# openclimatefix/predict_pv_yield

Measured on AMD Instinct MI355X. Metric: PV-site samples/sec (train step), conv3d 12->6 frames, higher is better.
Workload: dtype bf16; 1 GPU; conv3d train step (fwd + NMAE + bwd + Adam): sat [B,11,18,64,64] N(0,1), 4x Conv3d(3x3x3, 32ch) + fc 128/128/64, 128.6 M params; per_gpu_batch=32, global_batch=32, t_frames=18, parallelism=single

## Files before the change

### predict_pv_yield_amd/csrc/conv3d_wgrad_bf16_v2.hip

```cpp
#include "pv_common.h"

namespace pv {

constexpr int W2TR = 8, W2TRI = 10, W2TW = 32, W2XW = 34;
constexpr int W2_SLAB_ELEMS = 28 * 32 * 32;
constexpr uint32_t W2_INVALID = 0x40000000u;

typedef __attribute__((address_space(3))) s16x4 w2_lds_s16x4;
typedef __attribute__((address_space(3))) unsigned char* w2_lds_ptr;
typedef int w2_i32x4 __attribute__((ext_vector_type(4)));

__device__ __forceinline__ void w2_lds_dma16(uint32_t lds_addr, uint32_t voff, w2_i32x4 rsrc, uint32_t soff) {
  asm volatile("s_mov_b32 m0, %0\n\ts_nop 0\n\tbuffer_load_dwordx4 %1, %2, %3 offen lds" ::"s"(lds_addr), "v"(voff), "s"(rsrc),
               "s"(soff)
               : "memory");
}
__device__ __forceinline__ w2_i32x4 w2_rsrc(const void* base, int bytes) {
  const uintptr_t a = (uintptr_t)base;
  return (w2_i32x4){(int)(uint32_t)a, (int)((a >> 32) & 0xffffu), bytes, 0x00020000};
}

#ifdef PV_DIAG_STAMPS
__device__ unsigned long long wgrad2_diag[PV_DIAG_WAVES * PV_DIAG_SLOTS];
#endif

template <int NACC, int Q>
__device__ __forceinline__ void w2_interleave() {
  if constexpr (Q < NACC) {
    constexpr int R = 2 + 2 * NACC;
    __builtin_amdgcn_sched_group_barrier(0x008, 1, 0);
    __builtin_amdgcn_sched_group_barrier(0x100, R / NACC + (Q < R % NACC ? 1 : 0), 0);
    w2_interleave<NACC, Q + 1>();
  }
}

template <int CPAD, bool F16 = false, bool PACK12 = false>
__global__ __launch_bounds__(512, 2) void conv3d_wgrad_bf16_v2_kernel(
    const uint16_t* __restrict__ x, const uint16_t* __restrict__ dy, float* __restrict__ slabs, int t_in, int h_in, int w_in,
    int t_out, int h_out, int w_out, int pad_t, int pad_h, int pad_w, int n_colblk, int t_chunk, int rpb) {
  constexpr int NCH = CPAD / 8;
  constexpr int VPR = 16 / NCH;
  constexpr int VOXB = CPAD * 2;
  constexpr int ROWB = W2XW * VOXB;
  constexpr int SLOTB = W2TRI * ROWB;
  constexpr int XVPP = 1024 / VOXB;
  constexpr int XPIECES = (W2XW + XVPP - 1) / XVPP;
  constexpr int XTAIL_LANES = (W2XW - (XPIECES - 1) * XVPP) * NCH;
  constexpr int DROWB = W2TW * 64;
  constexpr int DSLOTB = W2TR * DROWB;
  constexpr int NXS = 5;
  __shared__ __attribute__((aligned(1024))) unsigned char lds[NXS * SLOTB + 256 + 2 * DSLOTB];
  unsigned char* lds_const = lds + NXS * SLOTB;
  unsigned char* lds_dy = lds_const + 256;

  const int tid = threadIdx.x;
  const int lane = tid & 63;
  const int wave8 = __builtin_amdgcn_readfirstlane(tid >> 6);
  const bool loader = wave8 >= 4;
  const int wave = wave8 & 3;
  const int grp = lane >> 4;
  const int qi = (lane & 15) >> 2;
  const int pi = lane & 3;
  const int hh = grp >> 1;
  const int cb = 16 * (grp & 1);

  const int h0 = blockIdx.x * rpb;
  const int b = blockIdx.z;
  const int tc0 = blockIdx.y * t_chunk;
  const int tc1 = min(tc0 + t_chunk, t_out);
  const int wg_id = (blockIdx.z * gridDim.y + blockIdx.y) * gridDim.x + blockIdx.x;
  float* slab = slabs + (size_t)wg_id * W2_SLAB_ELEMS;

  static_assert(!PACK12 || CPAD == 16, "PACK12 packs the 16-channel image");
  constexpr bool PAIRED = CPAD == 16;
  constexpr int NACC = PACK12 ? 3 : (PAIRED ? 4 : 7);
  f32x16 acc[NACC];
#pragma unroll
  for (int i = 0; i < NACC; ++i)
#pragma unroll
    for (int j = 0; j < 16; ++j) acc[i][j] = 0.f;

  const int nt = tc1 - tc0, tn = nt + 2;
  const int n_items = nt > 0 ? nt * n_colblk : 0;
  const int u_end = tn * n_colblk;
  const uint32_t lds_base = __builtin_amdgcn_readfirstlane((uint32_t)(uintptr_t)(w2_lds_ptr)lds);

  if (n_items > 0 && loader) {
    const uint32_t x_plane_b = (uint32_t)h_in * w_in * CPAD * 2u, x_row_b = (uint32_t)w_in * CPAD * 2u;
    const uint32_t d_plane_b = (uint32_t)h_out * w_out * 64u, d_row_b = (uint32_t)w_out * 64u;
    const size_t x_sample = (size_t)t_in * h_in * w_in * CPAD, d_sample = (size_t)t_out * h_out * w_out * 32;
    const void* const x_base = x + (size_t)b * x_sample;
    const void* const d_base = dy + (size_t)b * d_sample;
    const int x_bytes = (int)(x_sample * 2), d_bytes = (int)(d_sample * 2);
    uint32_t xrow_src[3];
    bool xrow_in[3];
#pragma unroll
    for (int i = 0; i < 3; ++i) {
      const int hi = h0 - pad_h + wave + 4 * i;
      xrow_in[i] = (unsigned)hi < (unsigned)h_in && wave + 4 * i < rpb + 2;
      xrow_src[i] = xrow_in[i] ? (uint32_t)hi * x_row_b : 0u;
    }
    uint32_t drow_src[2];
    bool drow_in[2];
#pragma unroll
    for (int i = 0; i < 2; ++i) {
      const int ho = h0 + wave + 4 * i;
      drow_in[i] = ho < h_out && wave + 4 * i < rpb;
      drow_src[i] = drow_in[i] ? (uint32_t)ho * d_row_b : 0u;
    }
    const bool has_third_row = wave + 8 < W2TRI;
    auto x_slice = [&](int u) {
      const int cb = u / tn, s = tc0 + (u - cb * tn), w0 = cb * W2TW;
      const int ti = s - pad_t;
      const bool t_ok = (unsigned)ti < (unsigned)t_in;
      const uint32_t slot = lds_base + (uint32_t)((u % NXS) * SLOTB);
#pragma unroll
      for (int pc = 0; pc < XPIECES; ++pc) {
        const int v = pc * XVPP + lane / NCH;
        const int src = (lane % NCH) ^ ((v / VPR) % NCH);
        const int wi = w0 - pad_w + v;
        const uint32_t lane_off = ((unsigned)wi < (unsigned)w_in && v < W2XW) ? (uint32_t)(wi * CPAD + src * 8) * 2u : W2_INVALID;
#pragma unroll
        for (int i = 0; i < 3; ++i) {
          if (i == 2 && !has_third_row) continue;
          const bool ok = t_ok && xrow_in[i];
          if (pc + 1 < XPIECES || lane < XTAIL_LANES)
            w2_lds_dma16(slot + (uint32_t)((wave + 4 * i) * ROWB + pc * 1024), lane_off, w2_rsrc(x_base, ok ? x_bytes : 0),
                         ok ? (uint32_t)ti * x_plane_b + xrow_src[i] : 0u);
        }
      }
    };
    auto d_slice = [&](int v_seq) {
      const int cb = v_seq / nt, t = tc0 + (v_seq - cb * nt), w0 = cb * W2TW;
      const uint32_t slot = lds_base + (uint32_t)(NXS * SLOTB + 256 + (v_seq & 1) * DSLOTB);
#pragma unroll
      for (int pc = 0; pc < 2; ++pc) {
        const int v = pc * 16 + (lane >> 2);
        const int src = (lane & 3) ^ ((v >> 2) & 3);
        const uint32_t lane_off = (w0 + v) < w_out ? (uint32_t)((w0 + v) * 32 + src * 8) * 2u : W2_INVALID;
#pragma unroll
        for (int i = 0; i < 2; ++i) {
          const bool ok = drow_in[i];
          w2_lds_dma16(slot + (uint32_t)((wave + 4 * i) * DROWB + pc * 1024), lane_off, w2_rsrc(d_base, ok ? d_bytes : 0),
                       ok ? (uint32_t)t * d_plane_b + drow_src[i] : 0u);
        }
      }
    };

    int next_u = 0;
    for (; next_u < 4 && next_u < u_end; ++next_u) x_slice(next_u);
    d_slice(0);
    for (int j = 0; j < n_items; ++j) {
      const int cb = j / nt, u0 = cb * tn + (j - cb * nt);
      __builtin_amdgcn_s_waitcnt(0x0f70);
      __syncthreads();
      if (next_u < u0 + 3) {
        for (; next_u < u0 + 3; ++next_u) x_slice(next_u);
        __builtin_amdgcn_s_waitcnt(0x0f70);
        __syncthreads();
      }
      for (; next_u <= u0 + 4 && next_u < u_end; ++next_u) x_slice(next_u);
      if (j + 1 < n_items) d_slice(j + 1);
    }
  } else if (n_items > 0) {
    if (tid < 64) reinterpret_cast<uint32_t*>(lds_const)[tid] = tid < 32 ? (F16 ? 0x3c003c00u : 0x3f803f80u) : 0u;

    int aoff[2];
#pragma unroll
    for (int s = 0; s < 2; ++s) {
      const int v = 8 * hh + 4 * s + qi;
      const int chunk = (cb + 4 * pi) >> 3;
      aoff[s] = v * 64 + ((chunk ^ ((v >> 2) & 3)) << 4) + (pi & 1) * 8;
    }
    int boff[NACC][2];
    int bkt[NACC];
    int my_tap[NACC];
#pragma unroll
    for (int i = 0; i < NACC; ++i) {
      int tap, c4 = 0;
      if constexpr (PACK12) {
        const int piece = 8 * (wave + 4 * i) + 4 * (grp & 1) + pi;
        tap = piece / 3;
        c4 = piece - 3 * tap;
        if (piece > 81) tap = 28;
      } else {
        tap = PAIRED ? 2 * (wave + 4 * i) + (grp & 1) : wave + 4 * i;
      }
      my_tap[i] = tap;
      if (tap > 26) tap = 26;
      const int kt = tap / 9, kh = (tap / 3) % 3, kw = tap % 3;
      bkt[i] = kt;
      const int cbx = PAIRED ? 0 : cb;
#pragma unroll
      for (int s = 0; s < 2; ++s) {
        const int v = kw + 8 * hh + 4 * s + qi;
        const int chunk = PACK12 ? (c4 >> 1) : ((cbx + 4 * pi) >> 3);
        const int sub = PACK12 ? (c4 & 1) : (pi & 1);
        boff[i][s] = kh * ROWB + v * VOXB + ((chunk ^ ((v / VPR) % NCH)) << 4) + sub * 8;
      }
    }
    typedef __attribute__((ext_vector_type(8))) short s16x8;
    const int last_tap = (PAIRED || PACK12) ? my_tap[NACC - 1] : (wave == 3 ? 27 : 0);
    const unsigned char* const_frag = last_tap < 27 ? nullptr : lds_const + (last_tap == 27 ? 0 : 128) + (lane & 15) * 8;

#ifdef PV_DIAG_STAMPS
    unsigned long long dg[PV_DIAG_SLOTS] = {0, 0, 0, 0, 0, 0, 0, 0}, s0, s1, s2;
#endif
    for (int j = 0; j < n_items; ++j) {
      const int cbj = j / nt, u0 = cbj * tn + (j - cbj * nt);
      PV_STAMP(s0);
      __syncthreads();
      if (cbj > 0 && j == cbj * nt) __syncthreads();
      PV_STAMP(s1);
      int slot_of_kt[3];
#pragma unroll
      for (int kt = 0; kt < 3; ++kt) slot_of_kt[kt] = ((u0 + kt) % NXS) * SLOTB;
      const unsigned char* dy_slot = lds_dy + (j & 1) * DSLOTB;
      int bslot[NACC];
#pragma unroll
      for (int i = 0; i < NACC; ++i) bslot[i] = bkt[i] == 0 ? slot_of_kt[0] : (bkt[i] == 1 ? slot_of_kt[1] : slot_of_kt[2]);
      auto read_step = [&](int st, s16x4 (&ra)[2], s16x4 (&rb)[NACC][2]) {
        const int rho = st >> 1, cg = st & 1;
        const unsigned char* ap = dy_slot + rho * DROWB + cg * 16 * 64;
        ra[0] = __builtin_amdgcn_ds_read_tr16_b64_v4i16((w2_lds_s16x4*)(ap + aoff[0]));
        ra[1] = __builtin_amdgcn_ds_read_tr16_b64_v4i16((w2_lds_s16x4*)(ap + aoff[1]));
        const int xo = rho * ROWB + cg * 16 * VOXB;
#pragma unroll
        for (int i = 0; i < NACC; ++i) {
          const unsigned char* bp = lds + bslot[i] + xo;
          const unsigned char* p0 = bp + boff[i][0];
          const unsigned char* p1 = bp + boff[i][1];
          if (i == NACC - 1) {
            p0 = const_frag ? const_frag : p0;
            p1 = const_frag ? const_frag : p1;
          }
          rb[i][0] = __builtin_amdgcn_ds_read_tr16_b64_v4i16((w2_lds_s16x4*)p0);
          rb[i][1] = __builtin_amdgcn_ds_read_tr16_b64_v4i16((w2_lds_s16x4*)p1);
        }
      };
      auto mfma_step = [&](const s16x4 (&ra)[2], const s16x4 (&rb)[NACC][2]) {
        const s16x8 a8 = {ra[0][0], ra[0][1], ra[0][2], ra[0][3], ra[1][0], ra[1][1], ra[1][2], ra[1][3]};
        typedef _Float16 w2_f16x8 __attribute__((ext_vector_type(8)));
#pragma unroll
        for (int i = 0; i < NACC; ++i) {
          s16x8 t8 = {rb[i][0][0], rb[i][0][1], rb[i][0][2], rb[i][0][3], rb[i][1][0], rb[i][1][1], rb[i][1][2], rb[i][1][3]};
          if constexpr (F16)
            acc[i] = __builtin_amdgcn_mfma_f32_32x32x16_f16(__builtin_bit_cast(w2_f16x8, a8), __builtin_bit_cast(w2_f16x8, t8), acc[i], 0, 0, 0);
          else
            acc[i] = __builtin_amdgcn_mfma_f32_32x32x16_bf16(__builtin_bit_cast(bf16x8, a8), __builtin_bit_cast(bf16x8, t8), acc[i], 0, 0, 0);
        }
      };
      s16x4 ra0[2], ra1[2], rb0[NACC][2], rb1[NACC][2];
      const bool skip_last_row = rpb < W2TR;
      read_step(0, ra0, rb0);
#pragma unroll
      for (int st = 0; st < W2TR * 2; st += 2) {
        if (st == W2TR * 2 - 2 && skip_last_row) break;
        __builtin_amdgcn_sched_barrier(0);
        read_step(st + 1, ra1, rb1);
        mfma_step(ra0, rb0);
        w2_interleave<NACC, 0>();
        __builtin_amdgcn_sched_barrier(0);
        if (st + 2 < W2TR * 2) {
          read_step(st + 2, ra0, rb0);
          mfma_step(ra1, rb1);
          w2_interleave<NACC, 0>();
        } else {
          mfma_step(ra1, rb1);
        }
        __builtin_amdgcn_sched_barrier(0);
      }
#ifdef PV_DIAG_STAMPS
      PV_STAMP(s2);
      dg[0] += s1 - s0;
      dg[1] += s2 - s1;
      dg[2] += 1;
#endif
    }
#ifdef PV_DIAG_STAMPS
    if (lane == 0 && wg_id * 4 + wave < PV_DIAG_WAVES)
      for (int i = 0; i < PV_DIAG_SLOTS; ++i) wgrad2_diag[(size_t)(wg_id * 4 + wave) * PV_DIAG_SLOTS + i] = dg[i];
#endif
  }
  if (loader) return;

  const int half = lane >> 5;
#pragma unroll
  for (int i = 0; i < NACC; ++i) {
    int tapslot = PAIRED ? 2 * (wave + 4 * i) + ((lane & 31) >> 4) : wave + 4 * i;
    int ci = PAIRED ? (lane & 15) : (lane & 31);
    if constexpr (PACK12) {
      const int piece = 8 * (wave + 4 * i) + ((lane & 31) >> 2);
      tapslot = piece / 3;
      ci = 4 * (piece - 3 * tapslot) + (lane & 3);
      if (piece > 81) tapslot = 28;
    }
    if (tapslot <= 27) {
      float* dst = slab + (size_t)tapslot * 1024 + ci;
#pragma unroll
      for (int j = 0; j < 16; ++j) {
        const int co = (j & 3) + 8 * (j >> 2) + 4 * half;
        dst[co * 32] = acc[i][j];
      }
    }
  }
}

void wgrad_v2_grid(const pv_conv3d_dims* d, int* n_rowblk, int* n_colblk, int* n_tchunk, int* t_chunk, int* rows_per_blk) {
  const int to = d->t_in + 2 * d->pad_t - 2, ho = d->h_in + 2 * d->pad_h - 2, wo = d->w_in + 2 * d->pad_w - 2;
  *n_rowblk = (ho + W2TR - 1) / W2TR;
  if ((long long)d->batch * *n_rowblk < 256 && (long long)d->batch * (*n_rowblk + 1) <= 256 &&
      (ho + *n_rowblk) / (*n_rowblk + 1) < (ho + *n_rowblk - 1) / *n_rowblk)
    *n_rowblk += 1;
  *rows_per_blk = (ho + *n_rowblk - 1) / *n_rowblk;
  *n_colblk = (wo + W2TW - 1) / W2TW;
  const long long tiles = (long long)d->batch * *n_rowblk;
  int max_chunks = (to + 1) / 2;
  if (max_chunks < 1) max_chunks = 1;
  int ntc = 1;
  long long best = -1;
  for (int c = 1; c <= max_chunks && tiles * c <= 16 * 256; ++c) {
    const int tch = (to + c - 1) / c, nch = (to + tch - 1) / tch;
    const long long rounds = (tiles * nch + 255) / 256;
    const long long cost = rounds * (tch + 2);
    if (best < 0 || cost < best) best = cost, ntc = nch;
  }
  *t_chunk = (to + ntc - 1) / ntc;
  *n_tchunk = (to + *t_chunk - 1) / *t_chunk;
}

size_t wgrad_v2_workspace_bytes(const pv_conv3d_dims* d) {
  int nrb, ncb, ntc, tch, rpb;
  wgrad_v2_grid(d, &nrb, &ncb, &ntc, &tch, &rpb);
  return (size_t)d->batch * nrb * ntc * W2_SLAB_ELEMS * sizeof(float);
}

int launch_conv3d_wgrad_bf16_v2(const uint16_t* x, const uint16_t* dy, float* slabs, const pv_conv3d_dims* d, int to, int ho,
                                int wo, hipStream_t st, int* n_slabs, bool f16) {
  if (((uintptr_t)x % 16) != 0 || ((uintptr_t)dy % 16) != 0) return 1;
  int nrb, ncb, ntc, tch, rpb;
  wgrad_v2_grid(d, &nrb, &ncb, &ntc, &tch, &rpb);
  *n_slabs = d->batch * nrb * ntc;
  dim3 grid((unsigned)nrb, (unsigned)ntc, (unsigned)d->batch);
#define PV_W2(CP, HALF)                                                                                                       \
  hipLaunchKernelGGL((conv3d_wgrad_bf16_v2_kernel<CP, HALF>), grid, dim3(512), 0, st, x, dy, slabs, d->t_in, d->h_in, d->w_in, to, \
                     ho, wo, d->pad_t, d->pad_h, d->pad_w, ncb, tch, rpb)
#define PV_W2P(HALF)                                                                                                        \
  hipLaunchKernelGGL((conv3d_wgrad_bf16_v2_kernel<16, HALF, true>), grid, dim3(512), 0, st, x, dy, slabs, d->t_in, d->h_in, d->w_in, \
                     to, ho, wo, d->pad_t, d->pad_h, d->pad_w, ncb, tch, rpb)
  if (pv_bf16_cpad(d->c_in) == 16) {
    const bool pack12 = d->c_in <= 12 && !getenv("PV_WGRAD_NO_PACK12");
    if (pack12) { if (f16) PV_W2P(true); else PV_W2P(false); }
    else { if (f16) PV_W2(16, true); else PV_W2(16, false); }
  } else { if (f16) PV_W2(32, true); else PV_W2(32, false); }
#undef PV_W2P
#undef PV_W2
  return 0;
}


constexpr int WR_GROUPS = 16;
__global__ __launch_bounds__(64 * WR_GROUPS) void conv3d_wgrad_reduce_kernel(const float* __restrict__ slabs, int n_slabs,
                                                                              float* __restrict__ dw, float* __restrict__ dbias,
                                                                              int c_out, int c_in) {
  __shared__ float part[WR_GROUPS][64];
  const int lane = threadIdx.x & 63, grp = threadIdx.x >> 6;
  const int i = blockIdx.x * 64 + lane;
  float s0 = 0.f, s1 = 0.f, s2 = 0.f, s3 = 0.f;
  for (int k = grp; k < n_slabs; k += 16 * WR_GROUPS) {
    float v[16];
#pragma unroll
    for (int j = 0; j < 16; ++j) v[j] = (k + WR_GROUPS * j < n_slabs) ? slabs[(size_t)(k + WR_GROUPS * j) * W2_SLAB_ELEMS + i] : 0.f;
#pragma unroll
    for (int j = 0; j < 16; j += 4) s0 += v[j], s1 += v[j + 1], s2 += v[j + 2], s3 += v[j + 3];
  }
  part[grp][lane] = (s0 + s1) + (s2 + s3);
  __syncthreads();
  if (grp == 0) {
    float t[WR_GROUPS];
#pragma unroll
    for (int q = 0; q < WR_GROUPS; ++q) t[q] = part[q][lane];
#pragma unroll
    for (int w = WR_GROUPS / 2; w >= 1; w >>= 1)
#pragma unroll
      for (int q = 0; q < w; ++q) t[q] = t[2 * q] + t[2 * q + 1];
    const float s = t[0];
    const int tap = i >> 10, co = (i >> 5) & 31, ci = i & 31;
    if (tap < 27) {
      if (dw && co < c_out && ci < c_in) dw[((size_t)co * c_in + ci) * 27 + tap] = s;
    } else if (dbias && ci == 0 && co < c_out) {
      dbias[co] = s;
    }
  }
}

__global__ __launch_bounds__(256) void wgrad_gate_copy_kernel(const u32x4* __restrict__ dy, const u32x4* __restrict__ y,
                                                              u32x4* __restrict__ dst, size_t n8) {
  const size_t stride = (size_t)gridDim.x * blockDim.x;
  for (size_t i = (size_t)blockIdx.x * blockDim.x + threadIdx.x; i < n8; i += stride) {
    const u32x4 g = dy[i], a = y[i];
    u32x4 o;
#pragma unroll
    for (int j = 0; j < 4; ++j) o[j] = g[j] & (relu_pair01(a[j]) * 0xffffu);
    dst[i] = o;
  }
}

}

using namespace pv;

extern "C" {

int pv_conv3d_bwd_weight_bf16_workspace_bytes(const pv_conv3d_dims* d, size_t* bytes) {
  PV_REQUIRE(d && bytes, PV_EINVAL, "pv_conv3d_bwd_weight_bf16_workspace_bytes: null pointer");
  PV_REQUIRE(d->batch > 0 && d->t_in > 0 && d->h_in > 0 && d->w_in > 0, PV_EINVAL,
             "pv_conv3d_bwd_weight_bf16_workspace_bytes: bad dims");
  const long long to = d->t_in + 2 * d->pad_t - 2, ho = d->h_in + 2 * d->pad_h - 2, wo = d->w_in + 2 * d->pad_w - 2;
  const size_t dy_bytes = (to > 0 && ho > 0 && wo > 0) ? (size_t)d->batch * to * ho * wo * pv_bf16_cpad(d->c_out) * 2 : 0;
  *bytes = ((wgrad_v2_workspace_bytes(d) + 255) & ~(size_t)255) + dy_bytes;
  return PV_OK;
}

int pv_conv3d_bwd_weight_bf16(const uint16_t* x, const uint16_t* dy, const uint16_t* y_relu_mask, float* dw,
                              float* dbias, const pv_conv3d_dims* d, void* workspace, size_t workspace_bytes,
                              void* stream) {
  PV_REQUIRE(d && x && dy && workspace, PV_EINVAL, "pv_conv3d_bwd_weight_bf16: null pointer");
  PV_REQUIRE(d->batch > 0 && d->c_in > 0 && d->c_in <= 32 && d->c_out > 0 && d->c_out <= 32, PV_ESIZE,
             "pv_conv3d_bwd_weight_bf16: channels (%d -> %d) must be in 1..32", d->c_in, d->c_out);
  PV_REQUIRE(d->pad_t >= 0 && d->pad_t <= 2 && d->pad_h >= 0 && d->pad_h <= 2 && d->pad_w >= 0 && d->pad_w <= 2,
             PV_EINVAL, "pv_conv3d_bwd_weight_bf16: padding must be 0..2");
  const int to = d->t_in + 2 * d->pad_t - 2, ho = d->h_in + 2 * d->pad_h - 2, wo = d->w_in + 2 * d->pad_w - 2;
  PV_REQUIRE(to > 0 && ho > 0 && wo > 0, PV_ESIZE, "pv_conv3d_bwd_weight_bf16: input smaller than the kernel");
  PV_REQUIRE(d->batch <= 65535, PV_ESIZE, "pv_conv3d_bwd_weight_bf16: batch too large for grid.z");
  PV_REQUIRE((size_t)d->t_in * d->h_in * d->w_in * 64 <= 0x40000000ull, PV_ESIZE,
             "pv_conv3d_bwd_weight_bf16: one sample exceeds 1 GiB (buffer-addressing limit of this kernel)");
  const size_t slab_bytes = (wgrad_v2_workspace_bytes(d) + 255) & ~(size_t)255;
  PV_REQUIRE(workspace_bytes >= wgrad_v2_workspace_bytes(d), PV_ESIZE, "pv_conv3d_bwd_weight_bf16: workspace too small");
  PV_REQUIRE(((uintptr_t)x % 16) == 0 && ((uintptr_t)dy % 16) == 0 && ((uintptr_t)workspace % 16) == 0, PV_EINVAL,
             "pv_conv3d_bwd_weight_bf16: x, dy and the workspace must be 16-byte aligned");
  hipStream_t st = as_stream(stream);
  if (y_relu_mask) {
    const size_t n = (size_t)d->batch * to * ho * wo * pv_bf16_cpad(d->c_out);
    PV_REQUIRE(workspace_bytes >= slab_bytes + n * 2, PV_ESIZE,
               "pv_conv3d_bwd_weight_bf16: a gate needs room for the gated copy of dY behind the slabs (workspace_bytes query)");
    PV_REQUIRE(((uintptr_t)y_relu_mask % 16) == 0, PV_EINVAL, "pv_conv3d_bwd_weight_bf16: the gate must be 16-byte aligned");
    uint16_t* gated = reinterpret_cast<uint16_t*>(static_cast<char*>(workspace) + slab_bytes);
    hipLaunchKernelGGL(wgrad_gate_copy_kernel, dim3(stream_grid(n / 8, 256)), dim3(256), 0, st,
                       reinterpret_cast<const u32x4*>(dy), reinterpret_cast<const u32x4*>(y_relu_mask),
                       reinterpret_cast<u32x4*>(gated), n / 8);
    dy = gated;
  }
  int n2 = 0;
  PV_REQUIRE(launch_conv3d_wgrad_bf16_v2(x, dy, (float*)workspace, d, to, ho, wo, st, &n2, false) == 0, PV_EINVAL,
             "pv_conv3d_bwd_weight_bf16: x and dy must be 16-byte aligned");
  hipLaunchKernelGGL(conv3d_wgrad_reduce_kernel, dim3(W2_SLAB_ELEMS / 64), dim3(64 * WR_GROUPS), 0, st, (const float*)workspace, n2,
                     dw, dbias, d->c_out, d->c_in);
  return check_launch("pv_conv3d_bwd_weight_bf16");
}

int pv_conv3d_bwd_weight_f16(const uint16_t* x, const uint16_t* dy, float* dw, float* dbias, const pv_conv3d_dims* d,
                             void* workspace, size_t workspace_bytes, void* stream) {
  PV_REQUIRE(d && x && dy && workspace, PV_EINVAL, "pv_conv3d_bwd_weight_f16: null pointer");
  PV_REQUIRE(d->batch > 0 && d->c_in > 0 && d->c_in <= 32 && d->c_out > 0 && d->c_out <= 32, PV_ESIZE,
             "pv_conv3d_bwd_weight_f16: channels (%d -> %d) must be in 1..32", d->c_in, d->c_out);
  PV_REQUIRE(d->pad_t >= 0 && d->pad_t <= 2 && d->pad_h >= 0 && d->pad_h <= 2 && d->pad_w >= 0 && d->pad_w <= 2,
             PV_EINVAL, "pv_conv3d_bwd_weight_f16: padding must be 0..2");
  const int to = d->t_in + 2 * d->pad_t - 2, ho = d->h_in + 2 * d->pad_h - 2, wo = d->w_in + 2 * d->pad_w - 2;
  PV_REQUIRE(to > 0 && ho > 0 && wo > 0, PV_ESIZE, "pv_conv3d_bwd_weight_f16: input smaller than the kernel");
  PV_REQUIRE(d->batch <= 65535, PV_ESIZE, "pv_conv3d_bwd_weight_f16: batch too large for grid.z");
  PV_REQUIRE((size_t)d->t_in * d->h_in * d->w_in * 64 <= 0x40000000ull, PV_ESIZE,
             "pv_conv3d_bwd_weight_f16: one sample exceeds 1 GiB (buffer-addressing limit of this kernel)");
  PV_REQUIRE(workspace_bytes >= wgrad_v2_workspace_bytes(d), PV_ESIZE, "pv_conv3d_bwd_weight_f16: workspace too small");
  hipStream_t st = as_stream(stream);
  int n2 = 0;
  PV_REQUIRE(launch_conv3d_wgrad_bf16_v2(x, dy, (float*)workspace, d, to, ho, wo, st, &n2, true) == 0, PV_EINVAL,
             "pv_conv3d_bwd_weight_f16: x and dy must be 16-byte aligned");
  hipLaunchKernelGGL(conv3d_wgrad_reduce_kernel, dim3(W2_SLAB_ELEMS / 64), dim3(64 * WR_GROUPS), 0, st, (const float*)workspace, n2,
                     dw, dbias, d->c_out, d->c_in);
  return check_launch("pv_conv3d_bwd_weight_f16");
}

}

#ifdef PV_DIAG_STAMPS
extern "C" int pv_diag_read_wgrad2(unsigned long long* host, size_t n) {
  return hipMemcpyFromSymbol(host, HIP_SYMBOL(pv::wgrad2_diag), n * sizeof(unsigned long long)) == hipSuccess ? 0 : -1;
}
#endif
```

Baseline: 19860 samples/s.

## Add v3 wgrad kernel with software-pipelined LDS transpose reads and MFMA interleave

Moves the loader-wave DMA staging into a shared helper and adds a new v3 weight-gradient kernel for 32-channel inputs, now the default path. Its compute waves use 32x32x16 MFMAs fed by ds_read_tr16 transpose loads, double-buffer fragments across steps and interleave LDS reads with MFMAs through sched_group_barriers. It also drops the last-row step when rows per block fall short of the tile height, and one wave uses a ones vector for the bias column instead of loading it. The aim is to hide LDS latency behind matrix work in the main wgrad loop, at the cost of more registers and scheduling rigidity.

```diff
diff --git a/predict_pv_yield_amd/csrc/conv3d_wgrad_bf16_v2.hip b/predict_pv_yield_amd/csrc/conv3d_wgrad_bf16_v2.hip
--- a/predict_pv_yield_amd/csrc/conv3d_wgrad_bf16_v2.hip
+++ b/predict_pv_yield_amd/csrc/conv3d_wgrad_bf16_v2.hip
@@ -31,6 +31,97 @@
     __builtin_amdgcn_sched_group_barrier(0x008, 1, 0);
     __builtin_amdgcn_sched_group_barrier(0x100, R / NACC + (Q < R % NACC ? 1 : 0), 0);
     w2_interleave<NACC, Q + 1>();
+  }
+}
+
+template <int CPAD>
+__device__ __forceinline__ void w2_stage(const uint16_t* __restrict__ x, const uint16_t* __restrict__ dy, uint32_t lds_base,
+                                         int b, int h0, int rpb, int tc0, int nt, int n_colblk, int wave, int lane, int t_in,
+                                         int h_in, int w_in, int t_out, int h_out, int w_out, int pad_t, int pad_h, int pad_w) {
+  constexpr int NCH = CPAD / 8, VPR = 16 / NCH, VOXB = CPAD * 2;
+  constexpr int ROWB = W2XW * VOXB, SLOTB = W2TRI * ROWB;
+  constexpr int XVPP = 1024 / VOXB;
+  constexpr int XPIECES = (W2XW + XVPP - 1) / XVPP;
+  constexpr int XTAIL_LANES = (W2XW - (XPIECES - 1) * XVPP) * NCH;
+  constexpr int DROWB = W2TW * 64, DSLOTB = W2TR * DROWB;
+  constexpr int NXS = 5;
+  const int tn = nt + 2, n_items = nt * n_colblk;
+  const int u_end = tn * n_colblk;
+  const uint32_t x_plane_b = (uint32_t)h_in * w_in * CPAD * 2u, x_row_b = (uint32_t)w_in * CPAD * 2u;
+  const uint32_t d_plane_b = (uint32_t)h_out * w_out * 64u, d_row_b = (uint32_t)w_out * 64u;
+  const size_t x_sample = (size_t)t_in * h_in * w_in * CPAD, d_sample = (size_t)t_out * h_out * w_out * 32;
+  const void* const x_base = x + (size_t)b * x_sample;
+  const void* const d_base = dy + (size_t)b * d_sample;
+  const int x_bytes = (int)(x_sample * 2), d_bytes = (int)(d_sample * 2);
+  uint32_t xrow_src[3];
+  bool xrow_in[3];
+#pragma unroll
+  for (int i = 0; i < 3; ++i) {
+    const int hi = h0 - pad_h + wave + 4 * i;
+    xrow_in[i] = (unsigned)hi < (unsigned)h_in && wave + 4 * i < rpb + 2;
+    xrow_src[i] = xrow_in[i] ? (uint32_t)hi * x_row_b : 0u;
+  }
+  uint32_t drow_src[2];
+  bool drow_in[2];
+#pragma unroll
+  for (int i = 0; i < 2; ++i) {
+    const int ho = h0 + wave + 4 * i;
+    drow_in[i] = ho < h_out && wave + 4 * i < rpb;
+    drow_src[i] = drow_in[i] ? (uint32_t)ho * d_row_b : 0u;
+  }
+  const bool has_third_row = wave + 8 < W2TRI;
+  auto x_slice = [&](int u) {
+    const int cb = u / tn, s = tc0 + (u - cb * tn), w0 = cb * W2TW;
+    const int ti = s - pad_t;
+    const bool t_ok = (unsigned)ti < (unsigned)t_in;
+    const uint32_t slot = lds_base + (uint32_t)((u % NXS) * SLOTB);
+#pragma unroll
+    for (int pc = 0; pc < XPIECES; ++pc) {
+      const int v = pc * XVPP + lane / NCH;
+      const int src = (lane % NCH) ^ ((v / VPR) % NCH);
+      const int wi = w0 - pad_w + v;
+      const uint32_t lane_off = ((unsigned)wi < (unsigned)w_in && v < W2XW) ? (uint32_t)(wi * CPAD + src * 8) * 2u : W2_INVALID;
+#pragma unroll
+      for (int i = 0; i < 3; ++i) {
+        if (i == 2 && !has_third_row) continue;
+        const bool ok = t_ok && xrow_in[i];
+        if (pc + 1 < XPIECES || lane < XTAIL_LANES)
+          w2_lds_dma16(slot + (uint32_t)((wave + 4 * i) * ROWB + pc * 1024), lane_off, w2_rsrc(x_base, ok ? x_bytes : 0),
+                       ok ? (uint32_t)ti * x_plane_b + xrow_src[i] : 0u);
+      }
+    }
+  };
+  auto d_slice = [&](int v_seq) {
+    const int cb = v_seq / nt, t = tc0 + (v_seq - cb * nt), w0 = cb * W2TW;
+    const uint32_t slot = lds_base + (uint32_t)(NXS * SLOTB + 256 + (v_seq & 1) * DSLOTB);
+#pragma unroll
+    for (int pc = 0; pc < 2; ++pc) {
+      const int v = pc * 16 + (lane >> 2);
+      const int src = (lane & 3) ^ ((v >> 2) & 3);
+      const uint32_t lane_off = (w0 + v) < w_out ? (uint32_t)((w0 + v) * 32 + src * 8) * 2u : W2_INVALID;
+#pragma unroll
+      for (int i = 0; i < 2; ++i) {
+        const bool ok = drow_in[i];
+        w2_lds_dma16(slot + (uint32_t)((wave + 4 * i) * DROWB + pc * 1024), lane_off, w2_rsrc(d_base, ok ? d_bytes : 0),
+                     ok ? (uint32_t)t * d_plane_b + drow_src[i] : 0u);
+      }
+    }
+  };
+
+  int next_u = 0;
+  for (; next_u < 4 && next_u < u_end; ++next_u) x_slice(next_u);
+  d_slice(0);
+  for (int j = 0; j < n_items; ++j) {
+    const int cb = j / nt, u0 = cb * tn + (j - cb * nt);
+    __builtin_amdgcn_s_waitcnt(0x0f70);
+    __syncthreads();
+    if (next_u < u0 + 3) {
+      for (; next_u < u0 + 3; ++next_u) x_slice(next_u);
+      __builtin_amdgcn_s_waitcnt(0x0f70);
+      __syncthreads();
+    }
+    for (; next_u <= u0 + 4 && next_u < u_end; ++next_u) x_slice(next_u);
+    if (j + 1 < n_items) d_slice(j + 1);
   }
 }
 
@@ -43,9 +134,6 @@
   constexpr int VOXB = CPAD * 2;
   constexpr int ROWB = W2XW * VOXB;
   constexpr int SLOTB = W2TRI * ROWB;
-  constexpr int XVPP = 1024 / VOXB;
-  constexpr int XPIECES = (W2XW + XVPP - 1) / XVPP;
-  constexpr int XTAIL_LANES = (W2XW - (XPIECES - 1) * XVPP) * NCH;
   constexpr int DROWB = W2TW * 64;
   constexpr int DSLOTB = W2TR * DROWB;
   constexpr int NXS = 5;
@@ -82,86 +170,11 @@
 
   const int nt = tc1 - tc0, tn = nt + 2;
   const int n_items = nt > 0 ? nt * n_colblk : 0;
-  const int u_end = tn * n_colblk;
   const uint32_t lds_base = __builtin_amdgcn_readfirstlane((uint32_t)(uintptr_t)(w2_lds_ptr)lds);
 
   if (n_items > 0 && loader) {
-    const uint32_t x_plane_b = (uint32_t)h_in * w_in * CPAD * 2u, x_row_b = (uint32_t)w_in * CPAD * 2u;
-    const uint32_t d_plane_b = (uint32_t)h_out * w_out * 64u, d_row_b = (uint32_t)w_out * 64u;
-    const size_t x_sample = (size_t)t_in * h_in * w_in * CPAD, d_sample = (size_t)t_out * h_out * w_out * 32;
-    const void* const x_base = x + (size_t)b * x_sample;
-    const void* const d_base = dy + (size_t)b * d_sample;
-    const int x_bytes = (int)(x_sample * 2), d_bytes = (int)(d_sample * 2);
-    uint32_t xrow_src[3];
-    bool xrow_in[3];
-#pragma unroll
-    for (int i = 0; i < 3; ++i) {
-      const int hi = h0 - pad_h + wave + 4 * i;
-      xrow_in[i] = (unsigned)hi < (unsigned)h_in && wave + 4 * i < rpb + 2;
-      xrow_src[i] = xrow_in[i] ? (uint32_t)hi * x_row_b : 0u;
-    }
-    uint32_t drow_src[2];
-    bool drow_in[2];
-#pragma unroll
-    for (int i = 0; i < 2; ++i) {
-      const int ho = h0 + wave + 4 * i;
-      drow_in[i] = ho < h_out && wave + 4 * i < rpb;
-      drow_src[i] = drow_in[i] ? (uint32_t)ho * d_row_b : 0u;
-    }
-    const bool has_third_row = wave + 8 < W2TRI;
-    auto x_slice = [&](int u) {
-      const int cb = u / tn, s = tc0 + (u - cb * tn), w0 = cb * W2TW;
-      const int ti = s - pad_t;
-      const bool t_ok = (unsigned)ti < (unsigned)t_in;
-      const uint32_t slot = lds_base + (uint32_t)((u % NXS) * SLOTB);
-#pragma unroll
-      for (int pc = 0; pc < XPIECES; ++pc) {
-        const int v = pc * XVPP + lane / NCH;
-        const int src = (lane % NCH) ^ ((v / VPR) % NCH);
-        const int wi = w0 - pad_w + v;
-        const uint32_t lane_off = ((unsigned)wi < (unsigned)w_in && v < W2XW) ? (uint32_t)(wi * CPAD + src * 8) * 2u : W2_INVALID;
-#pragma unroll
-        for (int i = 0; i < 3; ++i) {
-          if (i == 2 && !has_third_row) continue;
-          const bool ok = t_ok && xrow_in[i];
-          if (pc + 1 < XPIECES || lane < XTAIL_LANES)
-            w2_lds_dma16(slot + (uint32_t)((wave + 4 * i) * ROWB + pc * 1024), lane_off, w2_rsrc(x_base, ok ? x_bytes : 0),
-                         ok ? (uint32_t)ti * x_plane_b + xrow_src[i] : 0u);
-        }
-      }
-    };
-    auto d_slice = [&](int v_seq) {
-      const int cb = v_seq / nt, t = tc0 + (v_seq - cb * nt), w0 = cb * W2TW;
-      const uint32_t slot = lds_base + (uint32_t)(NXS * SLOTB + 256 + (v_seq & 1) * DSLOTB);
-#pragma unroll
-      for (int pc = 0; pc < 2; ++pc) {
-        const int v = pc * 16 + (lane >> 2);
-        const int src = (lane & 3) ^ ((v >> 2) & 3);
-        const uint32_t lane_off = (w0 + v) < w_out ? (uint32_t)((w0 + v) * 32 + src * 8) * 2u : W2_INVALID;
-#pragma unroll
-        for (int i = 0; i < 2; ++i) {
-          const bool ok = drow_in[i];
-          w2_lds_dma16(slot + (uint32_t)((wave + 4 * i) * DROWB + pc * 1024), lane_off, w2_rsrc(d_base, ok ? d_bytes : 0),
-                       ok ? (uint32_t)t * d_plane_b + drow_src[i] : 0u);
-        }
-      }
-    };
-
-    int next_u = 0;
-    for (; next_u < 4 && next_u < u_end; ++next_u) x_slice(next_u);
-    d_slice(0);
-    for (int j = 0; j < n_items; ++j) {
-      const int cb = j / nt, u0 = cb * tn + (j - cb * nt);
-      __builtin_amdgcn_s_waitcnt(0x0f70);
-      __syncthreads();
-      if (next_u < u0 + 3) {
-        for (; next_u < u0 + 3; ++next_u) x_slice(next_u);
-        __builtin_amdgcn_s_waitcnt(0x0f70);
-        __syncthreads();
-      }
-      for (; next_u <= u0 + 4 && next_u < u_end; ++next_u) x_slice(next_u);
-      if (j + 1 < n_items) d_slice(j + 1);
-    }
+    w2_stage<CPAD>(x, dy, lds_base, b, h0, rpb, tc0, nt, n_colblk, wave, lane, t_in, h_in, w_in, t_out, h_out, w_out, pad_t, pad_h,
+                   pad_w);
   } else if (n_items > 0) {
     if (tid < 64) reinterpret_cast<uint32_t*>(lds_const)[tid] = tid < 32 ? (F16 ? 0x3c003c00u : 0x3f803f80u) : 0u;
 
@@ -302,6 +315,194 @@
         const int co = (j & 3) + 8 * (j >> 2) + 4 * half;
         dst[co * 32] = acc[i][j];
       }
+    }
+  }
+}
+
+template <int NM, int NR, int Q = 0>
+__device__ __forceinline__ void w3_interleave() {
+  if constexpr (Q < NM) {
+    __builtin_amdgcn_sched_group_barrier(0x008, 1, 0);
+    constexpr int n = NR / NM + (Q < NR % NM ? 1 : 0);
+    if constexpr (n > 0) __builtin_amdgcn_sched_group_barrier(0x100, n, 0);
+    w3_interleave<NM, NR, Q + 1>();
+  }
+}
+template <int I, int N, class F>
+__device__ __forceinline__ void w3_static_for(F&& f) {
+  if constexpr (I < N) {
+    f(std::integral_constant<int, I>{});
+    w3_static_for<I + 1, N>(f);
+  }
+}
+
+template <bool F16, bool ONES>
+__device__ __forceinline__ void w3_multiply(f32x16 (&acc)[7], const unsigned char* lds, int wave, int lane, int n_items, int nt,
+                                            int tn, bool skip_last_row) {
+  constexpr int VOXB = 64, ROWB = W2XW * VOXB, SLOTB = W2TRI * ROWB, DROWB = W2TW * 64, DSLOTB = W2TR * DROWB, NXS = 5;
+  constexpr int NSTEP = W2TR * 2;
+  typedef __attribute__((ext_vector_type(8))) short s16x8;
+  typedef _Float16 w3_f16x8 __attribute__((ext_vector_type(8)));
+  const unsigned char* const lds_dy = lds + NXS * SLOTB + 256;
+  const int grp = lane >> 4, qi = (lane & 15) >> 2, pi = lane & 3, hh = grp >> 1, cb = 16 * (grp & 1);
+  const int chunk = (cb + 4 * pi) >> 3;
+  int aoff[2], goff[2][2], soff[2];
+  int gkt[2];
+#pragma unroll
+  for (int s = 0; s < 2; ++s) {
+    const int v = 8 * hh + 4 * s + qi;
+    aoff[s] = v * 64 + ((chunk ^ ((v >> 2) & 3)) << 4) + (pi & 1) * 8;
+  }
+  auto xoff = [&](int kw, int s) {
+    const int v = kw + 8 * hh + 4 * s + qi;
+    return v * VOXB + ((chunk ^ ((v >> 2) & 3)) << 4) + (pi & 1) * 8;
+  };
+#pragma unroll
+  for (int g = 0; g < 2; ++g) {
+    const int col = 2 * wave + g;
+    gkt[g] = col / 3;
+#pragma unroll
+    for (int s = 0; s < 2; ++s) goff[g][s] = xoff(col % 3, s);
+  }
+#pragma unroll
+  for (int s = 0; s < 2; ++s) soff[s] = wave * ROWB + xoff(2, s);
+  const short one = F16 ? (short)0x3c00 : (short)0x3f80;
+  const s16x8 ones = {one, one, one, one, one, one, one, one};
+
+#ifdef PV_DIAG_STAMPS
+  unsigned long long dg[PV_DIAG_SLOTS] = {0, 0, 0, 0, 0, 0, 0, 0}, s0, s1, s2;
+#endif
+  for (int j = 0; j < n_items; ++j) {
+    const int cbj = j / nt, u0 = cbj * tn + (j - cbj * nt);
+    PV_STAMP(s0);
+    __syncthreads();
+    if (cbj > 0 && j == cbj * nt) __syncthreads();
+    PV_STAMP(s1);
+    int slot_of_kt[3];
+#pragma unroll
+    for (int kt = 0; kt < 3; ++kt) slot_of_kt[kt] = ((u0 + kt) % NXS) * SLOTB;
+    const unsigned char* const dy_slot = lds_dy + (j & 1) * DSLOTB;
+    const unsigned char* ap[2];
+    const unsigned char* gp[2][2];
+    const unsigned char* sp[2];
+#pragma unroll
+    for (int s = 0; s < 2; ++s) {
+      ap[s] = dy_slot + aoff[s];
+      sp[s] = lds + slot_of_kt[2] + soff[s];
+#pragma unroll
+      for (int g = 0; g < 2; ++g) gp[g][s] = lds + (gkt[g] == 0 ? slot_of_kt[0] : (gkt[g] == 1 ? slot_of_kt[1] : slot_of_kt[2])) + goff[g][s];
+    }
+    s16x4 fa[2][2], fx[2][W2TRI][2][2], fs[2][2];
+    auto rd = [](const unsigned char* p) { return __builtin_amdgcn_ds_read_tr16_b64_v4i16((w2_lds_s16x4*)p); };
+    auto read_step = [&](auto st_c) {
+      constexpr int ST = decltype(st_c)::value, rho = ST >> 1, cg = ST & 1;
+#pragma unroll
+      for (int s = 0; s < 2; ++s) fa[ST & 1][s] = rd(ap[s] + rho * DROWB + cg * 1024);
+#pragma unroll
+      for (int r = rho == 0 ? 0 : rho + 2; r <= rho + 2; ++r) {
+#pragma unroll
+        for (int g = 0; g < 2; ++g)
+#pragma unroll
+          for (int s = 0; s < 2; ++s) fx[g][r][cg][s] = rd(gp[g][s] + r * ROWB + cg * 1024);
+        if constexpr (ST == 0) __builtin_amdgcn_sched_barrier(0);
+      }
+      if constexpr (!ONES)
+#pragma unroll
+        for (int s = 0; s < 2; ++s) fs[ST & 1][s] = rd(sp[s] + rho * ROWB + cg * 1024);
+    };
+    auto mfma = [&](int i, const s16x4 (&a)[2], const s16x8& b8) {
+      const s16x8 a8 = {a[0][0], a[0][1], a[0][2], a[0][3], a[1][0], a[1][1], a[1][2], a[1][3]};
+      if constexpr (F16)
+        acc[i] = __builtin_amdgcn_mfma_f32_32x32x16_f16(__builtin_bit_cast(w3_f16x8, a8), __builtin_bit_cast(w3_f16x8, b8), acc[i], 0, 0, 0);
+      else
+        acc[i] = __builtin_amdgcn_mfma_f32_32x32x16_bf16(__builtin_bit_cast(bf16x8, a8), __builtin_bit_cast(bf16x8, b8), acc[i], 0, 0, 0);
+    };
+    auto cat = [](const s16x4 (&f)[2]) {
+      return (s16x8){f[0][0], f[0][1], f[0][2], f[0][3], f[1][0], f[1][1], f[1][2], f[1][3]};
+    };
+    auto step = [&](auto st_c) {
+      constexpr int ST = decltype(st_c)::value, rho = ST >> 1, cg = ST & 1;
+      __builtin_amdgcn_sched_barrier(0);
+      if constexpr (ST + 1 < NSTEP) read_step(std::integral_constant<int, ST + 1>{});
+#pragma unroll
+      for (int kh = 0; kh < 3; ++kh)
+#pragma unroll
+        for (int g = 0; g < 2; ++g) mfma(3 * g + kh, fa[ST & 1], cat(fx[g][rho + kh][cg]));
+      mfma(6, fa[ST & 1], ONES ? ones : cat(fs[ST & 1]));
+      if constexpr (ST + 1 < NSTEP) {
+        constexpr int R1 = ST + 1 < 2 ? 14 : 6;
+        w3_interleave<7, R1 + (ONES ? 0 : 2)>();
+      }
+      __builtin_amdgcn_sched_barrier(0);
+    };
+    read_step(std::integral_constant<int, 0>{});
+    w3_static_for<0, NSTEP - 2>(step);
+    if (!skip_last_row) w3_static_for<NSTEP - 2, NSTEP>(step);
+#ifdef PV_DIAG_STAMPS
+    PV_STAMP(s2);
+    dg[0] += s1 - s0;
+    dg[1] += s2 - s1;
+    dg[2] += 1;
+#endif
+  }
+#ifdef PV_DIAG_STAMPS
+  const int wg_id = (blockIdx.z * gridDim.y + blockIdx.y) * gridDim.x + blockIdx.x;
+  if (lane == 0 && wg_id * 4 + wave < PV_DIAG_WAVES)
+    for (int i = 0; i < PV_DIAG_SLOTS; ++i) wgrad2_diag[(size_t)(wg_id * 4 + wave) * PV_DIAG_SLOTS + i] = dg[i];
+#endif
+}
+
+template <bool F16>
+__global__ __launch_bounds__(512, 2) void conv3d_wgrad_bf16_v3_kernel(
+    const uint16_t* __restrict__ x, const uint16_t* __restrict__ dy, float* __restrict__ slabs, int t_in, int h_in, int w_in,
+    int t_out, int h_out, int w_out, int pad_t, int pad_h, int pad_w, int n_colblk, int t_chunk, int rpb) {
+  constexpr int SLOTB = W2TRI * W2XW * 64, DSLOTB = W2TR * W2TW * 64;
+  __shared__ __attribute__((aligned(1024))) unsigned char lds[5 * SLOTB + 256 + 2 * DSLOTB];
+
+  const int tid = threadIdx.x;
+  const int lane = tid & 63;
+  const int wave8 = __builtin_amdgcn_readfirstlane(tid >> 6);
+  const bool loader = wave8 >= 4;
+  const int wave = wave8 & 3;
+  const int h0 = blockIdx.x * rpb;
+  const int b = blockIdx.z;
+  const int tc0 = blockIdx.y * t_chunk;
+  const int tc1 = min(tc0 + t_chunk, t_out);
+  const int wg_id = (blockIdx.z * gridDim.y + blockIdx.y) * gridDim.x + blockIdx.x;
+  float* slab = slabs + (size_t)wg_id * W2_SLAB_ELEMS;
+  const int nt = tc1 - tc0, tn = nt + 2;
+  const int n_items = nt > 0 ? nt * n_colblk : 0;
+  const uint32_t lds_base = __builtin_amdgcn_readfirstlane((uint32_t)(uintptr_t)(w2_lds_ptr)lds);
+
+  f32x16 acc[7];
+#pragma unroll
+  for (int i = 0; i < 7; ++i)
+#pragma unroll
+    for (int j = 0; j < 16; ++j) acc[i][j] = 0.f;
+  if (n_items > 0 && loader) {
+    w2_stage<32>(x, dy, lds_base, b, h0, rpb, tc0, nt, n_colblk, wave, lane, t_in, h_in, w_in, t_out, h_out, w_out, pad_t, pad_h,
+                 pad_w);
+  } else if (n_items > 0) {
+    if (wave == 3) w3_multiply<F16, true>(acc, lds, wave, lane, n_items, nt, tn, rpb < W2TR);
+    else w3_multiply<F16, false>(acc, lds, wave, lane, n_items, nt, tn, rpb < W2TR);
+  }
+  if (loader) return;
+
+  const int half = lane >> 5;
+#pragma unroll
+  for (int i = 0; i < 7; ++i) {
+    int tapslot;
+    if (i < 6) {
+      const int col = 2 * wave + i / 3;
+      tapslot = 9 * (col / 3) + 3 * (i % 3) + col % 3;
+    } else {
+      tapslot = wave < 3 ? 20 + 3 * wave : 27;
+    }
+    float* dst = slab + (size_t)tapslot * 1024 + (lane & 31);
+#pragma unroll
+    for (int j = 0; j < 16; ++j) {
+      const int co = (j & 3) + 8 * (j >> 2) + 4 * half;
+      dst[co * 32] = acc[i][j];
     }
   }
 }
@@ -348,11 +549,17 @@
 #define PV_W2P(HALF)                                                                                                        \
   hipLaunchKernelGGL((conv3d_wgrad_bf16_v2_kernel<16, HALF, true>), grid, dim3(512), 0, st, x, dy, slabs, d->t_in, d->h_in, d->w_in, \
                      to, ho, wo, d->pad_t, d->pad_h, d->pad_w, ncb, tch, rpb)
+#define PV_W3(HALF)                                                                                                         \
+  hipLaunchKernelGGL((conv3d_wgrad_bf16_v3_kernel<HALF>), grid, dim3(512), 0, st, x, dy, slabs, d->t_in, d->h_in, d->w_in, to, ho, \
+                     wo, d->pad_t, d->pad_h, d->pad_w, ncb, tch, rpb)
   if (pv_bf16_cpad(d->c_in) == 16) {
     const bool pack12 = d->c_in <= 12 && !getenv("PV_WGRAD_NO_PACK12");
     if (pack12) { if (f16) PV_W2P(true); else PV_W2P(false); }
     else { if (f16) PV_W2(16, true); else PV_W2(16, false); }
+  } else if (!getenv("PV_WGRAD_V2")) {
+    if (f16) PV_W3(true); else PV_W3(false);
   } else { if (f16) PV_W2(32, true); else PV_W2(32, false); }
+#undef PV_W3
 #undef PV_W2P
 #undef PV_W2
   return 0;
```

Result: no change. 20020 samples/s (median of 6 runs) (+0.8%).
